# JohnsonLabJanelia/laserCalib

Hardware: NVIDIA B200
Metric: LM_iters_per_sec (higher is better)
Workload: dtype f64

## Files before the change

### include/lcba.h

```cpp
#ifndef LCBA_H
#define LCBA_H

#include <stddef.h>
#include <stdint.h>

#ifdef __cplusplus
extern "C" {
#endif

#define LCBA_VERSION 100
#define LCBA_CAM_PARAMS 11
#define LCBA_MAX_CAMERAS 64
#define LCBA_MAX_TRACE 512

enum {
  LCBA_OK = 0,
  LCBA_E_ARG = -1,
  LCBA_E_CUDA = -2,
  LCBA_E_STATE = -3,
  LCBA_E_UNSUPPORTED = -4,
  LCBA_E_NONFINITE = -5,
  LCBA_E_NCCL = -6
};

// ... 100 lines not shown

int lcba_nccl_unique_id(void* id_out128);
int lcba_comm_init(lcba_t* h, int32_t rank, int32_t nranks, const void* id128);

int lcba_debug_tr2d(double B00, double B01, double B11, double g0, double g1, double Delta,
                    double* p_out2, int* newton_out);

int lcba_debug_chol(lcba_t* h, int32_t n, const double* A, const double* rhs, double mu, const double* d,
                    int32_t grid, double* x_out, double* factor_out, int32_t* fail_out);

#define LCBA_STEP_SCALARS 18
int lcba_debug_step(lcba_t* h, double lam, double mu, int32_t mode, double* pc_out, double* pp_out,
                    double* scalars_out);

int lcba_debug_schur_stats(lcba_t* h, long long* out, int max_ctas, int* nkinds, int* nslices);

int lcba_debug_mma_plan(int32_t C, int32_t sm_count, int32_t* units_out, int32_t max_kinds,
                        int32_t* nslices_out, int32_t* ok_out);

int lcba_debug_i8_plan(int32_t C, int64_t P, int32_t sm_count, int32_t* tiles_out, int32_t max_tiles,
                       int32_t* work_out, int32_t max_work, int32_t* nwork_out, int32_t* nrg_out,
                       int64_t* nkb_out);

int lcba_debug_i8_fallback(lcba_t* h);

int lcba_debug_peer_reduce(lcba_t* h, int enable);

int lcba_host_is_nondecreasing_i64(const int64_t* v, int64_t n, int32_t threads);

#ifdef __cplusplus
}
#endif
#endif
```

### lasercalib_b200/_cabi.py

```python
from __future__ import annotations

import ctypes as C
import os

import numpy as np

_PKG = os.path.dirname(os.path.abspath(__file__))
LIB_PATH = os.path.join(_PKG, "liblcba.so")

LCBA_MAX_TRACE = 512
E_NAMES = {-1: "LCBA_E_ARG", -2: "LCBA_E_CUDA", -3: "LCBA_E_STATE", -4: "LCBA_E_UNSUPPORTED",
           -5: "LCBA_E_NONFINITE", -6: "LCBA_E_NCCL"}

SYMBOLS = ["lcba_version", "lcba_create", "lcba_destroy", "lcba_last_error", "lcba_default_options",
           "lcba_set_problem", "lcba_set_problem_shard", "lcba_set_params", "lcba_get_params", "lcba_rotate", "lcba_project",
           "lcba_unproject", "lcba_residuals", "lcba_jacobian_blocks", "lcba_sparsity_indices", "lcba_solve",
           "lcba_get_trace", "lcba_get_grad", "lcba_get_profile", "lcba_linearize",
           "lcba_time_device", "lcba_nccl_unique_id", "lcba_comm_init", "lcba_debug_tr2d",
           "lcba_sq_normal", "lcba_debug_schur_stats", "lcba_debug_mma_plan",
           "lcba_set_iteration_callback", "lcba_debug_i8_plan", "lcba_host_is_nondecreasing_i64", "lcba_debug_peer_reduce",
           "lcba_debug_i8_fallback", "lcba_debug_chol", "lcba_debug_step"]

STEP_SCALARS = ["reg_term", "Delta", "Jg2", "aa", "ab", "bb", "JAA", "JAB", "JBB", "gtgt", "gtp", "pp",
                "c0", "c1", "predicted", "step_h_norm", "step_norm", "chol_fail"]


class Options(C.Structure):
    _fields_ = [("ftol", C.c_double), ("xtol", C.c_double), ("gtol", C.c_double),
                ("max_nfev", C.c_int64), ("verbose", C.c_int32), ("profile", C.c_int32),
                ("max_iterations", C.c_int32), ("fix_cameras", C.c_int32), ("shared_intrinsics", C.c_int32), ("reserved", C.c_int32 * 3)]


class TraceRow(C.Structure):
    _fields_ = [("iteration", C.c_int64), ("nfev", C.c_int64), ("cost", C.c_double),
                ("cost_reduction", C.c_double), ("step_norm", C.c_double),
                ("optimality", C.c_double), ("delta", C.c_double), ("reg_term", C.c_double)]


class Result(C.Structure):
    _fields_ = [("cost", C.c_double), ("optimality", C.c_double), ("initial_cost", C.c_double),
                ("nfev", C.c_int64), ("njev", C.c_int64), ("iterations", C.c_int64),
                ("status", C.c_int32), ("n_trace", C.c_int32), ("solve_ms", C.c_double),
                ("gpu_launches", C.c_int64), ("reserved", C.c_double * 6)]

# ... 44 lines not shown
    lib.lcba_get_params.argtypes = [vp, vp, vp]
    lib.lcba_rotate.argtypes = [vp, i64, vp, vp, vp]
    lib.lcba_project.argtypes = [vp, i64, vp, vp, vp]
    lib.lcba_unproject.argtypes = [vp, i64, vp, vp, i64, vp, vp, vp, vp, vp]
    lib.lcba_residuals.argtypes = [vp, vp, vp, pd]
    lib.lcba_jacobian_blocks.argtypes = [vp, vp, vp, vp]
    lib.lcba_sparsity_indices.argtypes = [vp, i32, i64, i64, vp, vp, vp]
    lib.lcba_solve.argtypes = [vp, C.POINTER(Options), C.POINTER(Result)]
    lib.lcba_get_trace.argtypes = [vp, C.POINTER(TraceRow), i32]
    lib.lcba_set_iteration_callback.argtypes = [vp, ITERATION_CB, vp]
    lib.lcba_get_grad.argtypes = [vp, vp]
    lib.lcba_get_profile.argtypes = [vp, C.POINTER(KernelStat), i32, C.POINTER(i32)]
    lib.lcba_linearize.argtypes = [vp, dbl, vp, vp, vp, vp, pd]
    lib.lcba_time_device.argtypes = [vp, i32, i32, pd]
    lib.lcba_nccl_unique_id.argtypes = [vp]
    lib.lcba_comm_init.argtypes = [vp, i32, i32, vp]
    lib.lcba_sq_normal.argtypes = [vp, i32, vp, pd, vp, vp]
    lib.lcba_debug_mma_plan.argtypes = [i32, i32, vp, i32, C.POINTER(i32), C.POINTER(i32)]
    lib.lcba_debug_schur_stats.argtypes = [vp, vp, C.c_int, C.POINTER(C.c_int), C.POINTER(C.c_int)]
    lib.lcba_debug_i8_plan.argtypes = [i32, i64, i32, vp, i32, vp, i32, C.POINTER(i32), C.POINTER(i32), C.POINTER(i64)]
    lib.lcba_host_is_nondecreasing_i64.argtypes = [vp, i64, i32]
    lib.lcba_debug_peer_reduce.argtypes = [vp, i32]
    lib.lcba_debug_i8_fallback.argtypes = [vp]
    lib.lcba_debug_tr2d.argtypes = [dbl, dbl, dbl, dbl, dbl, dbl, pd, C.POINTER(C.c_int)]
    lib.lcba_debug_chol.argtypes = [vp, i32, vp, vp, dbl, vp, i32, vp, vp, C.POINTER(i32)]
    lib.lcba_debug_step.argtypes = [vp, dbl, dbl, i32, vp, vp, vp]
    _lib = lib
    return lib


def _ptr(a):
    return None if a is None else a.ctypes.data_as(C.c_void_p)


def _f64(a, shape=None):
    a = np.ascontiguousarray(a, dtype=np.float64)
    if shape is not None:
        a = a.reshape(shape)
    return a


def _i64(a):
    return np.ascontiguousarray(a, dtype=np.int64)


class Engine:
# ... 158 lines not shown
        return g

    def profile(self):
        stats = (KernelStat * 64)()
        n = C.c_int32()
        self._check(self.lib.lcba_get_profile(self.h, stats, 64, C.byref(n)))
        return {s.name.decode(): dict(launches=s.launches, total_ms=s.total_ms)
                for s in stats[:n.value]}

    def linearize(self, lam):
        n = 11 * self.C
        S = np.empty((n, n))
        rhs = np.empty(n)
        g = np.empty(n + 3 * self.P)
        sc = np.empty(n + 3 * self.P)
        cost = C.c_double()
        self._check(self.lib.lcba_linearize(self.h, float(lam), _ptr(S), _ptr(rhs), _ptr(g),
                                            _ptr(sc), C.byref(cost)))
        return dict(S=S, rhs=rhs, grad=g, scale_inv=sc, cost=cost.value)

    def i8_fell_back(self):
        return self.lib.lcba_debug_i8_fallback(self.h)

    def debug_chol(self, A, rhs, mu=0.0, d=None, grid=0):
        A = _f64(A)
        n = A.shape[0]
        if A.shape != (n, n):
            raise ValueError("A must be square")
        rhs = _f64(rhs).ravel()
        d = None if d is None else _f64(d).ravel()
        if rhs.size != n or (d is not None and d.size != n):
            raise ValueError("rhs and d must have n entries")
        x = np.empty(n)
        factor = np.empty((n + 1, n))
        fail = C.c_int32()
        self._check(self.lib.lcba_debug_chol(self.h, n, _ptr(A), _ptr(rhs), float(mu), _ptr(d), int(grid),
                                             _ptr(x), _ptr(factor), C.byref(fail)))
        return x, factor, fail.value

    STEP_FULL, STEP_FIX_CAMERAS, STEP_SHARED_INTRINSICS = 0, 1, 2

    def debug_step(self, lam, mu=0.0, mode=0):
        pc = np.empty(11 * self.C)
        pp = np.empty(3 * self.P)
        sc = np.empty(len(STEP_SCALARS))
        self._check(self.lib.lcba_debug_step(self.h, float(lam), float(mu), int(mode), _ptr(pc), _ptr(pp), _ptr(sc)))
# ... 28 lines not shown
```

### lasercalib_b200/csrc/lcba.cu

```cuda
#include <dlfcn.h>
#include <math.h>
#include <stdio.h>
#include <string.h>
#include <algorithm>
#include <map>
#include <string>
#include <thread>
#include <vector>

#include <nvtx3/nvToolsExt.h>

#include "common.cuh"
#include "control.cuh"
#include "dense.cuh"
#include "eval.cuh"
#include "ingest.cuh"
#include "linearize.cuh"
#include "dense_passes.cuh"
#include "schur.cuh"
#include "schur_mma.cuh"
#include "schur_i8.cuh"
#include "peer_reduce.cuh"
#include "variants.cuh"

// ... 504 lines not shown
  h->plan = make_schur_plan(C, h->sm_count, h->smem_optin - 2048);
  LCBA_TRY(dev_alloc(h, &h->d_kinds, h->plan.kinds.size()));
  LCBA_TRY(dev_alloc(h, &h->d_hws, h->plan.hws.size()));
  LCBA_CUDA(h, cudaMemcpyAsync(h->d_kinds, h->plan.kinds.data(), h->plan.kinds.size() * sizeof(SchurKind),
                               cudaMemcpyHostToDevice, st));
  LCBA_CUDA(h, cudaMemcpyAsync(h->d_hws, h->plan.hws.data(), h->plan.hws.size() * sizeof(SchurHw),
                               cudaMemcpyHostToDevice, st));
  LCBA_TRY(dev_alloc(h, &h->d_Sred, h->plan.part_stride));
  h->use_mma = false;
  h->d_mkinds = nullptr; h->d_U = nullptr; h->d_Upart = nullptr; h->d_Yg = nullptr;
  int max_slices = h->plan.nslices;
  {
    const char* de = getenv("LCBA_MMA_DENSITY");
    const double min_density = de ? atof(de) : 0.25;
    const bool dense = (double)h->n_pairs >= min_density * (double)P * C;
    const char* env = getenv("LCBA_SCHUR_MMA");
    const bool want = env ? atoi(env) != 0 : (dense && C >= 8);
    if (want && C <= MMA_MAX_CAMERAS) {
      {
        const char* ie = getenv("LCBA_SCHUR_I8");
        h->use_i8 = ie ? atoi(ie) != 0 : P >= 32768;
      }
      if (h->use_i8) {
        h->i8plan = make_i8_plan(C, P, h->sm_count);
        const I8Plan& ip = h->i8plan;
        h->i8_groups = (C + I8_GROUP_CAMS - 1) / I8_GROUP_CAMS;
        h->i8_gx_max = (int)std::max<long long>(1, std::min<long long>(ip.nkb, (long long)h->sm_count * 4 / h->i8_groups));
        h->i8_gx_make = (int)std::max<long long>(1, std::min<long long>(ip.nkb, (long long)h->sm_count * 3 / h->i8_groups));
        LCBA_TRY(dev_alloc(h, &h->d_i8work, ip.work.size()));
        LCBA_TRY(dev_alloc(h, &h->d_i8tiles, ip.tiles.size()));
        LCBA_CUDA(h, cudaMemcpyAsync(h->d_i8work, ip.work.data(), ip.work.size() * sizeof(I8Work), cudaMemcpyHostToDevice, st));
        LCBA_CUDA(h, cudaMemcpyAsync(h->d_i8tiles, ip.tiles.data(), ip.tiles.size() * sizeof(I8Tile), cudaMemcpyHostToDevice, st));
        LCBA_TRY(dev_alloc(h, &h->d_i8planes, ip.plane_bytes));
        {
          const char* te = getenv("LCBA_I8_TMA");
          h->i8_tma = !(te && atoi(te) == 0) && i8_encode_maps(ip, h->d_i8planes, &h->i8maps);
          if (!h->i8_tma) memset(&h->i8maps, 0, sizeof(h->i8maps));
        }
        LCBA_TRY(dev_alloc(h, &h->d_i8partial, ip.work.size() * 128 * 64));
        LCBA_TRY(dev_alloc(h, &h->d_i8rmax, (size_t)h->i8_gx_max * ip.NRG * 8));
        LCBA_TRY(dev_alloc(h, &h->d_i8erow, (size_t)ip.NRG * 8));
        LCBA_TRY(dev_alloc(h, &h->d_i8gate, 1));
        LCBA_TRY(dev_alloc(h, &h->d_i8mrow, (size_t)ip.NRG * 8));
        LCBA_CUDA(h, cudaMemsetAsync(h->d_i8gate, 0, sizeof(int), st));
        {
          const char* ge = getenv("LCBA_I8_GUARD");
          h->i8_guard = !(ge && atoi(ge) == 0);
// ... 326 lines not shown
  KL(h, "point_factor", k_point_factor<<<nblk(h->P, 256), 256, 0, h->stream>>>(
        h->d_Vg, h->d_scl_p, lam_arg, ctl_arg, h->P, h->d_Lz));
  if (h->use_mma) {
    const MmaPlan& mp = h->mplan;
    if (!h->use_dense) {
    const size_t smem_u = ((size_t)((C * CAMTAB + 1) & ~1) + (size_t)h->camn_pb * C) * 8;
    KL(h, "cam_normal", k_cam_normal<<<h->camn_grid, 256, smem_u, h->stream>>>(
          h->d_tab[w], h->d_pts[w], h->d_pair_w, h->d_pair_start, h->d_mask, h->P, C, h->camn_pb, h->d_Upart));
    KL(h, "reduce", k_reduce_cols<<<nblk(C * CAMN_VALS, RC_COLS), RC_COLS * RC_ROWS, 0, h->stream>>>(
          h->d_Upart, h->camn_grid, C * CAMN_VALS, h->d_U));
    }
    const int nt = (NCP * C + 1 + 7) / 8, last = nt - 6 * ((nt + 5) / 6 - 1);
    if (h->use_i8) {
      const I8Plan& ip = h->i8plan;
      const int RP = ip.NRG * 8;
      const size_t smem_rm = ((size_t)I8_GROUP_CAMS * CAMTAB + 192) * 4;
      KL(h, "i8_rowmax", k_i8_rowmax<<<dim3(h->i8_gx_max, h->i8_groups), 192, smem_rm, h->stream>>>(
            h->d_tab[w], h->d_pts[w], h->d_pair_w, h->d_pair_start, h->d_mask, h->d_Lz, h->P, C, RP, h->d_i8rmax));
      KL(h, "i8_rowmax", k_i8_rowexp<<<nblk(RP, 128), 128, 0, h->stream>>>(h->d_i8rmax, h->i8_gx_max, NCP * C + 1, RP,
                                                                     h->d_i8erow, h->d_i8mrow));
      KL(h, "make_Y", k_i8_make<<<dim3(h->i8_gx_make, h->i8_groups), 192, i8_make_smem_bytes(), h->stream>>>(
            h->d_tab[w], h->d_pts[w], h->d_pair_w, h->d_pair_start, h->d_mask, h->d_Lz, h->P, C, ip.NRG, h->d_i8erow,
            h->d_i8planes));
      if (h->i8_tma)
        KL(h, "schur", k_i8_syrk<true><<<(unsigned)ip.work.size(), I8_THREADS, ip.smem_bytes, h->stream>>>(
              h->i8maps, h->d_i8planes, ip.NRG, h->d_i8work, h->d_i8partial, h->d_fail, h->d_stats));
      else
        KL(h, "schur", k_i8_syrk<false><<<(unsigned)ip.work.size(), I8_THREADS, ip.smem_bytes, h->stream>>>(
              h->i8maps, h->d_i8planes, ip.NRG, h->d_i8work, h->d_i8partial, h->d_fail, h->d_stats));
      KL(h, "schur_reduce", k_i8_gather<<<dim3((unsigned)ip.tiles.size(), 16), 256, 0, h->stream>>>(
            h->d_i8partial, h->d_i8tiles, C, h->d_i8erow, pl.npairs, h->d_Sred));
      KL(h, "schur_reduce", k_add_cam_blocks<<<nblk(C * 121, 128), 128, 0, h->stream>>>(h->d_U, C, h->d_Sred));
      if (h->i8_guard) {
        KL(h, "i8_check", k_i8_check<<<1, 256, 0, h->stream>>>(h->d_i8mrow, C, h->d_Sred, h->d_i8gate));
#define LCBA_MMA_GATED(L)                                                                            \
  KL(h, "i8_fallback", (k_schur_mma<L, false><<<dim3(mp.nslices, mp.nkinds), MMA_THREADS, mp.smem_bytes, h->stream>>>( \
          nullptr, h->d_tab[w], h->d_pts[w], h->d_pair_w, h->d_pair_start, h->d_mask, h->d_Lz, h->P, h->n_pairs, C, \
          h->d_mkinds, mp.nslices, pl.part_stride, pl.npairs, h->d_Spart, nullptr, h->d_i8gate)))
        switch (last) {
          case 1: LCBA_MMA_GATED(1); break;
          case 2: LCBA_MMA_GATED(2); break;
          case 3: LCBA_MMA_GATED(3); break;
          case 4: LCBA_MMA_GATED(4); break;
          case 5: LCBA_MMA_GATED(5); break;
          default: LCBA_MMA_GATED(6); break;
        }
#undef LCBA_MMA_GATED
        KL(h, "i8_fallback", k_i8_fallback_finish<<<h->sm_count, 256, 0, h->stream>>>(
              h->d_i8gate, h->d_Spart, mp.nslices, pl.part_stride, h->d_U, C, h->d_Sred));
      }
// ... 631 lines not shown
      cudaMemcpy(&v, h->d_i8gate, sizeof(int), cudaMemcpyDeviceToHost) != cudaSuccess) return -1;
  return v;
}

extern "C" int lcba_debug_mma_plan(int32_t C, int32_t sm_count, int32_t* units_out, int32_t max_kinds,
                                   int32_t* nslices_out, int32_t* ok_out) {
  if (C < 1 || C > LCBA_MAX_CAMERAS || !units_out) return LCBA_E_ARG;
  const MmaPlan pl = make_mma_plan(C, sm_count, 227 * 1024 - 2048);
  if (ok_out) *ok_out = (pl.nkinds > 0 && C <= MMA_MAX_CAMERAS) ? 1 : 0;
  if (nslices_out) *nslices_out = pl.nslices;
  for (int k = 0; k < pl.nkinds && k < max_kinds; ++k)
    for (int w = 0; w < MMA_CONS_WARPS; ++w) {
      const MmaUnit& u = pl.kinds[k].unit[w];
      int32_t* o = units_out + ((size_t)k * MMA_CONS_WARPS + w) * 5;
      o[0] = u.tr0; o[1] = u.tc0; o[2] = u.nr; o[3] = u.nc; o[4] = u.tri;
    }
  return pl.nkinds;
}

extern "C" int lcba_debug_i8_plan(int32_t C, int64_t P, int32_t sm_count, int32_t* tiles_out, int32_t max_tiles,
                                  int32_t* work_out, int32_t max_work, int32_t* nwork_out, int32_t* nrg_out,
                                  int64_t* nkb_out) {
  if (C < 1 || C > LCBA_MAX_CAMERAS || P < 1 || !tiles_out) return LCBA_E_ARG;
  const I8Plan pl = make_i8_plan(C, P, sm_count);
  for (size_t i = 0; i < pl.tiles.size() && (int)i < max_tiles; ++i) {
    const I8Tile& t = pl.tiles[i];
    int32_t* o = tiles_out + 8 * i;
    o[0] = t.m_rg0; o[1] = t.m_nrg; o[2] = t.n_rg0; o[3] = t.n_nrg; o[4] = t.n2_rg0; o[5] = t.n2_nrg; o[6] = t.w0; o[7] = t.nw;
  }
  if (work_out)
    for (size_t i = 0; i < pl.work.size() && (int)i < max_work; ++i) {
      work_out[3 * i] = (int32_t)i; work_out[3 * i + 1] = pl.work[i].kb0; work_out[3 * i + 2] = pl.work[i].kb1;
    }
  if (nwork_out) *nwork_out = (int32_t)pl.work.size();
  if (nrg_out) *nrg_out = pl.NRG;
  if (nkb_out) *nkb_out = pl.nkb;
  return (int)pl.tiles.size();
}

extern "C" int lcba_sq_normal(lcba_t* h, int32_t mode, const double* theta, double* cost_out,
                              double* g_out, double* H_out) {
  if (!h || !h->have_problem) { set_error(h, "lcba_sq_normal: no problem set"); return LCBA_E_STATE; }
  if (!theta || (mode != LCBA_SQ_CAMONLY && mode != LCBA_SQ_TRANSFORM) || ((g_out == nullptr) != (H_out == nullptr))) {
    set_error(h, "lcba_sq_normal: bad mode, NULL theta, or only one of g / H given");
    return LCBA_E_ARG;
  }
  cudaSetDevice(h->device);
  const int C = h->C;
  const bool derivs = g_out != nullptr;
  const int K = (mode == LCBA_SQ_CAMONLY ? C * SQC_VALS : SQT_VALS) + 1;
  const int warps = sq_camonly_warps(C, h->smem_optin);
  const int threads = (mode == LCBA_SQ_CAMONLY) ? warps * 32 : SQ_THREADS;
  const int per_sm = (mode == LCBA_SQ_CAMONLY) ? 1 : 2;
  const int grid = (int)std::max<long long>(1, std::min<long long>((h->N + threads - 1) / threads,
                                                                   (long long)h->sm_count * per_sm));
  if (!h->d_sqpart || h->sq_grid < grid || h->sq_K < K) {
    LCBA_TRY(dev_alloc(h, &h->d_sqpart, (size_t)grid * K));
    LCBA_TRY(dev_alloc(h, &h->d_sqout, (size_t)K));
    if (!h->d_theta) LCBA_TRY(dev_alloc(h, &h->d_theta, 16));
    h->sq_grid = grid;
// ... 173 lines not shown
```

### lasercalib_b200/csrc/schur_i8.cuh

```cuda
#pragma once
#include <cuda.h>
#include <algorithm>
#include <vector>
#include "common.cuh"
#include "schur_mma.cuh"

namespace lcba {

constexpr int I8_NS = 6;
constexpr int I8_DMAX = 6;
constexpr int I8_ND = I8_DMAX + 1;
constexpr int I8_PTS = 21;
constexpr int I8_STAGES = 3;
constexpr int I8_FLUSH = 224;
constexpr int I8_THREADS = 192;
constexpr int I8_RG_BYTES = 512;
constexpr int I8_GROUP_CAMS = 8;
constexpr int I8_GROUP_RG = 13;
constexpr int I8_GROUP_ROWS = I8_GROUP_RG * 8;

struct I8Work {
  int m_rg0, m_nrg, n_rg0, n_nrg, n2_rg0, n2_nrg;
  int kb0, kb1;
  int map_a, map_b1, map_b2, pad;
};
constexpr int I8_MAX_MAPS = 6;
struct alignas(64) I8Maps { CUtensorMap m[I8_MAX_MAPS]; };
struct I8Tile { int m_rg0, m_nrg, n_rg0, n_nrg, n2_rg0, n2_nrg, w0, nw; };

struct I8Plan {
  int C = 0, R = 0, NRG = 0;
  long long nkb = 0;
  int map_heights[I8_MAX_MAPS] = {0, 0, 0, 0, 0, 0};
  int nmaps = 0;
  std::vector<I8Tile> tiles;
  std::vector<I8Work> work;
  size_t plane_bytes = 0, smem_bytes = 0;
};

inline I8Plan make_i8_plan(int C, long long P, int sm_count) {
  I8Plan pl;
  pl.C = C;
  pl.R = NCP * C + 1;
  pl.NRG = (pl.R + 7) / 8;
  pl.NRG += pl.NRG & 1;
  pl.nkb = (P + I8_PTS - 1) / I8_PTS;
  const int NRG = pl.NRG;
  const int nmt = (NRG + 15) / 16;
  const int last_m = NRG - 16 * (nmt - 1);
  const bool fold = nmt > 1 && last_m <= 4;
  const int nfull = fold ? nmt - 1 : nmt;
  const int col_w = fold ? 8 - last_m : 8;
  const int c0 = 16 * (nmt - 1);
  for (int mt = 0; mt < nfull; ++mt) {
    const int m0 = 16 * mt, mn = std::min(16, NRG - m0);
    for (int n0 = 0; n0 < m0 + mn; n0 += col_w) {
      const int nn = std::min(col_w, m0 + mn - n0);
      const bool last = n0 + col_w >= m0 + mn;
      I8Tile t{m0, mn, n0, nn, fold && last ? c0 : 0, fold && last ? last_m : 0, 0, 0};
      pl.tiles.push_back(t);
    }
  }
  if (fold) {
    I8Tile t{c0, last_m, c0, last_m, 0, 0, 0, 0};
    pl.tiles.push_back(t);
  }
  auto block_cost = [](int nrg) { return nrg <= 0 ? 0.0 : (nrg <= 2 ? 592.0 : (nrg <= 4 ? 812.0 : (nrg <= 6 ? 1181.0 : 1550.0))); };
  std::vector<double> cost(pl.tiles.size());
  std::vector<long long> nr(pl.tiles.size(), 1);
  for (size_t ti = 0; ti < pl.tiles.size(); ++ti) cost[ti] = 507.0 + block_cost(pl.tiles[ti].n_nrg) + block_cost(pl.tiles[ti].n2_nrg);
  for (long long left = (long long)sm_count - (long long)pl.tiles.size(); left > 0; --left) {
    size_t worst = 0;
    double tw = -1.0;
    for (size_t ti = 0; ti < pl.tiles.size(); ++ti) {
      const double tt = nr[ti] < pl.nkb ? cost[ti] / (double)nr[ti] : -1.0;
      if (tt > tw) { tw = tt; worst = ti; }
    }
    if (tw < 0.0) break;
    ++nr[worst];
  }
  for (size_t ti = 0; ti < pl.tiles.size(); ++ti) {
    I8Tile& t = pl.tiles[ti];
    const long long n = std::min<long long>(nr[ti], pl.nkb);
    t.w0 = (int)pl.work.size();
    t.nw = (int)n;
    auto map_of = [&](int h) {
      if (h == 0) return 0;
      for (int i = 0; i < pl.nmaps && i < I8_MAX_MAPS; ++i) if (pl.map_heights[i] == h) return i;
      if (pl.nmaps < I8_MAX_MAPS) pl.map_heights[pl.nmaps] = h;
      return pl.nmaps++;
    };
    const int ma = map_of(t.m_nrg), mb1 = map_of(t.n_nrg), mb2 = map_of(t.n2_nrg);
    for (long long q = 0; q < n; ++q) {
      I8Work w{t.m_rg0, t.m_nrg, t.n_rg0, t.n_nrg, t.n2_rg0, t.n2_nrg, (int)(pl.nkb * q / n), (int)(pl.nkb * (q + 1) / n),
               ma, mb1, mb2, 0};
      pl.work.push_back(w);
    }
  }
  pl.plane_bytes = (size_t)pl.nkb * I8_NS * NRG * I8_RG_BYTES;
  pl.smem_bytes = (size_t)I8_STAGES * I8_NS * (16 + 8) * I8_RG_BYTES + 1024;
  return pl;
}

inline bool i8_encode_maps(const I8Plan& pl, void* planes, I8Maps* out) {
  if (pl.nmaps <= 0 || pl.nmaps > I8_MAX_MAPS) return false;
  typedef CUresult (*EncodeFn)(CUtensorMap*, CUtensorMapDataType, cuuint32_t, void*, const cuuint64_t*, const cuuint64_t*,
                               const cuuint32_t*, const cuuint32_t*, CUtensorMapInterleave, CUtensorMapSwizzle,
                               CUtensorMapL2promotion, CUtensorMapFloatOOBfill);
  void* fn = nullptr;
  cudaDriverEntryPointQueryResult qres;
  if (cudaGetDriverEntryPoint("cuTensorMapEncodeTiled", &fn, cudaEnableDefault, &qres) != cudaSuccess || !fn ||
      qres != cudaDriverEntryPointSuccess) {
    cudaGetLastError();
    return false;
  }
  const cuuint64_t gdim[4] = {128, (cuuint64_t)pl.NRG, (cuuint64_t)I8_NS, (cuuint64_t)pl.nkb};
  const cuuint64_t gstr[3] = {(cuuint64_t)I8_RG_BYTES, (cuuint64_t)pl.NRG * I8_RG_BYTES, (cuuint64_t)I8_NS * pl.NRG * I8_RG_BYTES};
  const cuuint32_t estr[4] = {1, 1, 1, 1};
  memset(out, 0, sizeof(*out));
  for (int i = 0; i < pl.nmaps; ++i) {
    const cuuint32_t box[4] = {128, (cuuint32_t)pl.map_heights[i], (cuuint32_t)I8_NS, 1};
    const CUresult r = ((EncodeFn)fn)(&out->m[i], CU_TENSOR_MAP_DATA_TYPE_UINT32, 4, planes, gdim, gstr, box, estr,
                                      CU_TENSOR_MAP_INTERLEAVE_NONE, CU_TENSOR_MAP_SWIZZLE_NONE,
                                      CU_TENSOR_MAP_L2_PROMOTION_L2_256B, CU_TENSOR_MAP_FLOAT_OOB_FILL_NONE);
    if (r != CUDA_SUCCESS) return false;
  }
  return true;
}

__device__ __forceinline__ void i8_tma_4d(uint32_t dst, const CUtensorMap* map, int c0, int c1, int c2, int c3, uint32_t bar) {
  asm volatile("cp.async.bulk.tensor.4d.shared::cluster.global.mbarrier::complete_tx::bytes [%0], [%1, {%2, %3, %4, %5}], [%6];"
               ::"r"(dst), "l"(map), "r"(c0), "r"(c1), "r"(c2), "r"(c3), "r"(bar) : "memory");
}
__device__ __forceinline__ uint32_t i8_smem_u32(const void* p) { return (uint32_t)__cvta_generic_to_shared(p); }
__device__ __forceinline__ void i8_mbar_init(uint32_t bar, uint32_t count) {
  asm volatile("mbarrier.init.shared::cta.b64 [%0], %1;" ::"r"(bar), "r"(count) : "memory");
}
__device__ __forceinline__ void i8_mbar_expect_tx(uint32_t bar, uint32_t bytes) {
  asm volatile("mbarrier.arrive.expect_tx.shared::cta.b64 _, [%0], %1;" ::"r"(bar), "r"(bytes) : "memory");
}
__device__ __forceinline__ void i8_mbar_arrive(uint32_t bar) {
  asm volatile("mbarrier.arrive.shared::cta.b64 _, [%0];" ::"r"(bar) : "memory");
}
template <bool BACKOFF>
__device__ __forceinline__ void i8_mbar_wait(uint32_t bar, uint32_t parity, int* fail) {
  const long long t0 = clock64();
  while (true) {
    uint32_t ok;
    asm volatile("{\n\t.reg .pred p;\n\tmbarrier.try_wait.parity.shared::cta.b64 p, [%1], %2;\n\tselp.u32 %0, 1, 0, p;\n\t}"
                 : "=r"(ok) : "r"(bar), "r"(parity) : "memory");
    if (ok) return;
    if (BACKOFF) __nanosleep(128);
    if (clock64() - t0 > 6000000000LL) { atomicOr(fail, 4); asm volatile("trap;"); }
  }
}
__device__ __forceinline__ void i8_bulk_g2s(uint32_t dst, const void* src, uint32_t bytes, uint32_t bar) {
  asm volatile("cp.async.bulk.shared::cluster.global.mbarrier::complete_tx::bytes [%0], [%1], %2, [%3];"
               ::"r"(dst), "l"(src), "r"(bytes), "r"(bar) : "memory");
}
template <int COLL>
__device__ __forceinline__ void i8_mma(uint32_t tmem_d, uint64_t adesc, uint64_t bdesc, uint32_t idesc, uint32_t acc) {
#define I8_MMA_ASM(Q)                                                                                      \
  asm volatile("{\n\t.reg .pred p;\n\tsetp.ne.b32 p, %4, 0;\n\t"                                          \
               "tcgen05.mma.cta_group::1.kind::i8" Q " [%0], %1, %2, %3, {%5, %5, %5, %5}, p;\n\t}"         \
               ::"r"(tmem_d), "l"(adesc), "l"(bdesc), "r"(idesc), "r"(acc), "r"(0u) : "memory")
  if (COLL == 1) I8_MMA_ASM(".collector::a::fill");
  else if (COLL == 2) I8_MMA_ASM(".collector::a::use");
  else if (COLL == 3) I8_MMA_ASM(".collector::a::lastuse");
  else I8_MMA_ASM("");
#undef I8_MMA_ASM
}
__device__ __forceinline__ void i8_commit(uint32_t bar) {
  asm volatile("tcgen05.commit.cta_group::1.mbarrier::arrive::one.shared::cluster.b64 [%0];" ::"r"(bar) : "memory");
}
__device__ __forceinline__ bool i8_elect_one() {
  uint32_t p;
  asm volatile("{\n\t.reg .pred q;\n\telect.sync _|q, 0xffffffff;\n\tselp.u32 %0, 1, 0, q;\n\t}" : "=r"(p));
  return p != 0;
}
__device__ __forceinline__ void i8_tmem_ld16(uint32_t taddr, uint32_t (&v)[16]) {
  asm volatile("tcgen05.ld.sync.aligned.32x32b.x16.b32 "
               "{%0, %1, %2, %3, %4, %5, %6, %7, %8, %9, %10, %11, %12, %13, %14, %15}, [%16];"
               : "=r"(v[0]), "=r"(v[1]), "=r"(v[2]), "=r"(v[3]), "=r"(v[4]), "=r"(v[5]), "=r"(v[6]), "=r"(v[7]),
                 "=r"(v[8]), "=r"(v[9]), "=r"(v[10]), "=r"(v[11]), "=r"(v[12]), "=r"(v[13]), "=r"(v[14]), "=r"(v[15])
               : "r"(taddr) : "memory");
}

__device__ __forceinline__ void i8_item_values(const double* __restrict__ T, const double (&X)[3],
                                               const double (&li)[9], double w, bool live, double (&y)[3][NCP]) {
  ObsLin L;
  obs_linearize<false>(T, X[0], X[1], X[2], 0.0, 0.0, w, L, live);
  double Q[2][3];
#pragma unroll
  for (int i = 0; i < 2; ++i) {
    Q[i][0] = L.Jp[i][0] * li[0];
    Q[i][1] = fma(L.Jp[i][0], li[1], L.Jp[i][1] * li[2]);
// ... 320 lines not shown
    }
  }
}

template <bool TMA>
__global__ void __launch_bounds__(I8_THREADS, 1)
k_i8_syrk(const __grid_constant__ I8Maps maps, const unsigned char* __restrict__ planes, int NRG,
          const I8Work* __restrict__ work, double* __restrict__ partial, int* __restrict__ fail,
          long long* __restrict__ stats ) {
  extern __shared__ __align__(1024) uint8_t i8_smem[];
  __shared__ __align__(8) uint64_t s_bar[2 * I8_STAGES + 2];
  __shared__ uint32_t s_tmem;
  const I8Work W = work[blockIdx.x];
  const int tid = threadIdx.x, wid = tid >> 5, lane = tid & 31;
  const uint32_t a_bytes = (uint32_t)W.m_nrg * I8_RG_BYTES, b_bytes = (uint32_t)W.n_nrg * I8_RG_BYTES;
  const uint32_t b2_bytes = (uint32_t)W.n2_nrg * I8_RG_BYTES;
  const uint32_t B2_OFF = (uint32_t)I8_NS * b_bytes;
  constexpr uint32_t A_REGION = (uint32_t)I8_NS * 16 * I8_RG_BYTES;
  constexpr uint32_t STAGE_BYTES = (uint32_t)I8_NS * (16 + 8) * I8_RG_BYTES;
  const uint32_t smem0 = i8_smem_u32(i8_smem);
  const uint32_t bar_full = i8_smem_u32(&s_bar[0]), bar_empty = i8_smem_u32(&s_bar[I8_STAGES]);
  const uint32_t bar_tfull = i8_smem_u32(&s_bar[2 * I8_STAGES]), bar_tempty = i8_smem_u32(&s_bar[2 * I8_STAGES + 1]);
  const int ncol = W.n_nrg * 8, ncol2 = W.n2_nrg * 8;
  if (tid == 0) {
    for (int s = 0; s < I8_STAGES; ++s) { i8_mbar_init(bar_full + 8 * s, 1); i8_mbar_init(bar_empty + 8 * s, 1); }
    i8_mbar_init(bar_tfull, 1);
    i8_mbar_init(bar_tempty, 128);
    asm volatile("fence.mbarrier_init.release.cluster;" ::: "memory");
  }
  if (wid == 5) {
    asm volatile("tcgen05.alloc.cta_group::1.sync.aligned.shared::cta.b32 [%0], %1;" ::"r"(i8_smem_u32(&s_tmem)), "r"(512u) : "memory");
    asm volatile("tcgen05.relinquish_alloc_permit.cta_group::1.sync.aligned;" ::: "memory");
  }
  asm volatile("tcgen05.fence::before_thread_sync;" ::: "memory");
  __syncthreads();
  asm volatile("tcgen05.fence::after_thread_sync;" ::: "memory");
  const uint32_t tmem = s_tmem;
  const int nkb = W.kb1 - W.kb0;

  if (wid == 4) {
    if (TMA) {
      if (lane == 0) {
        for (int it = 0; it < nkb; ++it) {
          const int st = it % I8_STAGES;
          if (it >= I8_STAGES) i8_mbar_wait<false>(bar_empty + 8 * st, ((it / I8_STAGES) - 1) & 1, fail);
          i8_mbar_expect_tx(bar_full + 8 * st, (uint32_t)I8_NS * (a_bytes + b_bytes + b2_bytes));
          const uint32_t dstA = smem0 + st * STAGE_BYTES, dstB = dstA + A_REGION;
          const int kb = W.kb0 + it;
          i8_tma_4d(dstA, &maps.m[W.map_a], 0, W.m_rg0, 0, kb, bar_full + 8 * st);
          i8_tma_4d(dstB, &maps.m[W.map_b1], 0, W.n_rg0, 0, kb, bar_full + 8 * st);
          if (W.n2_nrg > 0) i8_tma_4d(dstB + B2_OFF, &maps.m[W.map_b2], 0, W.n2_rg0, 0, kb, bar_full + 8 * st);
        }
      }
    } else {
    const int ci = lane / 3, cb = lane - 3 * ci;
    const bool mine = lane < 3 * I8_NS && (cb < 2 || W.n2_nrg > 0);
    for (int it = 0; it < nkb; ++it) {
      const int st = it % I8_STAGES;
      if (it >= I8_STAGES) i8_mbar_wait<false>(bar_empty + 8 * st, ((it / I8_STAGES) - 1) & 1, fail);
      if (lane == 0) i8_mbar_expect_tx(bar_full + 8 * st, (uint32_t)I8_NS * (a_bytes + b_bytes + b2_bytes));
      __syncwarp();
      if (mine) {
        const unsigned char* src = planes + (size_t)(W.kb0 + it) * I8_NS * NRG * I8_RG_BYTES + (size_t)ci * NRG * I8_RG_BYTES;
        const uint32_t dstA = smem0 + st * STAGE_BYTES, dstB = dstA + A_REGION;
        if (cb == 0) i8_bulk_g2s(dstA + ci * a_bytes, src + (size_t)W.m_rg0 * I8_RG_BYTES, a_bytes, bar_full + 8 * st);
        else if (cb == 1) i8_bulk_g2s(dstB + ci * b_bytes, src + (size_t)W.n_rg0 * I8_RG_BYTES, b_bytes, bar_full + 8 * st);
        else i8_bulk_g2s(dstB + B2_OFF + ci * b2_bytes, src + (size_t)W.n2_rg0 * I8_RG_BYTES, b2_bytes, bar_full + 8 * st);
      }
    }
    }
  } else if (wid == 5) {
    if (i8_elect_one()) {
      int since_flush = 0, nflush = 0;
      long long t_wait = 0;
      const long long t_begin = stats ? clock64() : 0;
// ... 7 lines not shown
          const long long w0 = clock64();
          i8_mbar_wait<false>(bar_full + 8 * st, (it / I8_STAGES) & 1, fail);
          t_wait += clock64() - w0;
        } else {
          i8_mbar_wait<false>(bar_full + 8 * st, (it / I8_STAGES) & 1, fail);
        }
        asm volatile("tcgen05.fence::after_thread_sync;" ::: "memory");
        const uint32_t sA = smem0 + st * STAGE_BYTES, sB = sA + A_REGION;
        const bool first = since_flush == 0;
        const uint32_t sB2 = sB + B2_OFF;
        if (ncol2 == 0) {
          if (ncol == 64) i8_issue_block<64, 0>(first, tmem, sA, sB, sB2, a_bytes, b_bytes, b2_bytes);
          else if (ncol == 48) i8_issue_block<48, 0>(first, tmem, sA, sB, sB2, a_bytes, b_bytes, b2_bytes);
          else if (ncol == 32) i8_issue_block<32, 0>(first, tmem, sA, sB, sB2, a_bytes, b_bytes, b2_bytes);
          else i8_issue_block<16, 0>(first, tmem, sA, sB, sB2, a_bytes, b_bytes, b2_bytes);
        } else if (ncol2 == 16) {
          if (ncol == 48) i8_issue_block<48, 16>(first, tmem, sA, sB, sB2, a_bytes, b_bytes, b2_bytes);
          else if (ncol == 32) i8_issue_block<32, 16>(first, tmem, sA, sB, sB2, a_bytes, b_bytes, b2_bytes);
          else i8_issue_block<16, 16>(first, tmem, sA, sB, sB2, a_bytes, b_bytes, b2_bytes);
        } else {
          if (ncol == 32) i8_issue_block<32, 32>(first, tmem, sA, sB, sB2, a_bytes, b_bytes, b2_bytes);
          else i8_issue_block<16, 32>(first, tmem, sA, sB, sB2, a_bytes, b_bytes, b2_bytes);
        }
        i8_commit(bar_empty + 8 * st);
        ++since_flush;
        if (since_flush == I8_FLUSH || it == nkb - 1) {
          i8_commit(bar_tfull);
          since_flush = 0;
          ++nflush;
        }
      }
      if (stats) { stats[4 * blockIdx.x] = t_wait; stats[4 * blockIdx.x + 1] = clock64() - t_begin; }
    }
  } else {
    const int q = wid & 3;
    const int row = q * 32 + lane;
    double acc[64];
#pragma unroll
    for (int c = 0; c < 64; ++c) acc[c] = 0.0;
    const int nfl = (nkb + I8_FLUSH - 1) / I8_FLUSH;
    for (int f = 0; f < nfl; ++f) {
      i8_mbar_wait<true>(bar_tfull, f & 1, fail);
      asm volatile("tcgen05.fence::after_thread_sync;" ::: "memory");
#pragma unroll 1
      for (int d = 0; d < I8_ND; ++d) {
        const double sc = ldexp(1.0, -8 * (d + 2));
        const uint32_t taddr = tmem + ((uint32_t)(q * 32) << 16) + (uint32_t)(d * ncol);
#pragma unroll
        for (int h = 0; h < 4; ++h) {
          if (16 * h < ncol) {
            uint32_t v[16];
            i8_tmem_ld16(taddr + 16 * h, v);
            asm volatile("tcgen05.wait::ld.sync.aligned;" ::: "memory");
#pragma unroll
            for (int c = 0; c < 16; ++c) acc[16 * h + c] = fma((double)(int)v[c], sc, acc[16 * h + c]);
          } else if (16 * h >= 64 - ncol2) {
            uint32_t v[16];
            i8_tmem_ld16(tmem + ((uint32_t)(q * 32) << 16) + (uint32_t)(I8_ND * ncol + d * ncol2 + 16 * h - (64 - ncol2)), v);
            asm volatile("tcgen05.wait::ld.sync.aligned;" ::: "memory");
#pragma unroll
            for (int c = 0; c < 16; ++c) acc[16 * h + c] = fma((double)(int)v[c], sc, acc[16 * h + c]);
          }
        }
      }
      asm volatile("tcgen05.fence::before_thread_sync;" ::: "memory");
      i8_mbar_arrive(bar_tempty);
    }
    double* out = partial + ((size_t)blockIdx.x * 128 + row) * 64;
#pragma unroll
    for (int c = 0; c < 64; ++c) out[c] = acc[c];
  }
  asm volatile("tcgen05.fence::before_thread_sync;" ::: "memory");
  __syncthreads();
  if (wid == 5) asm volatile("tcgen05.dealloc.cta_group::1.sync.aligned.b32 %0, %1;" ::"r"(tmem), "r"(512u) : "memory");
}

__global__ void __launch_bounds__(256)
k_i8_gather(const double* __restrict__ partial, const I8Tile* __restrict__ tiles, int C,
            const int* __restrict__ e_row, int npairs, double* __restrict__ Sred) {
  const I8Tile T = tiles[blockIdx.x];
  const int n = NCP * C;
  const int nr = T.m_nrg * 8, nc1 = T.n_nrg * 8, nc2 = T.n2_nrg * 8, nc = nc1 + nc2;
  for (int idx = threadIdx.x + blockDim.x * blockIdx.y; idx < nr * nc; idx += blockDim.x * gridDim.y) {
    const int tr = idx / nc, tcl = idx - tr * nc;
    const bool second = tcl >= nc1;
    const int tc = second ? 64 - nc2 + (tcl - nc1) : tcl;
    int rho = T.m_rg0 * 8 + tr, sig = second ? T.n2_rg0 * 8 + (tcl - nc1) : T.n_rg0 * 8 + tcl;
    if (second) { const int x = rho; rho = sig; sig = x; }
    if (rho > n || sig >= n || sig > rho) continue;
    double s = 0.0;
    for (int w = 0; w < T.nw; ++w) s += partial[((size_t)(T.w0 + w) * 128 + tr) * 64 + tc];
    const double v = -ldexp(s, e_row[rho] + e_row[sig]);
    const int ck = sig / NCP, cb = sig % NCP;
    if (rho == n) { Sred[(size_t)npairs * 121 + ck * NCP + cb] = v; continue; }
    const int cj = rho / NCP, ra = rho % NCP;
    double* blk = Sred + (size_t)(cj * (cj + 1) / 2 + ck) * 121;
// ... 45 lines not shown
```

Before: 127.7.

## Multicast shared A-operand across CTA clusters and add TMA L2 prefetch in i8 SYRK

The int8 Schur SYRK kernel now pairs work items that share the same row tile and launches them as 2-CTA clusters. Each CTA loads half of the A-operand digit planes and multicasts them to its partner, and the empty barriers are signalled across the cluster with multicast commits. A TMA L2 prefetch that runs several k-blocks ahead is also added. The aim is to cut global/L2 traffic for the A operand and hide load latency. In exchange it adds cluster synchronisation, needs a scheduling check that falls back to non-clustered launches, and couples paired CTAs so that one stalls when the other does.

```diff
diff --git a/include/lcba.h b/include/lcba.h
--- a/include/lcba.h
+++ b/include/lcba.h
@@ -146,6 +146,11 @@
                        int32_t* work_out, int32_t max_work, int32_t* nwork_out, int32_t* nrg_out,
                        int64_t* nkb_out);
 
+int lcba_debug_i8_clusters(int32_t C, int64_t P, int32_t sm_count, int32_t max_cluster, int32_t* work_out,
+                           int32_t max_work, int32_t* nwork_out, int32_t* nmaps_out, int64_t* kb_bytes_out);
+
+int lcba_debug_i8_route(lcba_t* h);
+
 int lcba_debug_i8_fallback(lcba_t* h);
 
 int lcba_debug_peer_reduce(lcba_t* h, int enable);
diff --git a/lasercalib_b200/_cabi.py b/lasercalib_b200/_cabi.py
--- a/lasercalib_b200/_cabi.py
+++ b/lasercalib_b200/_cabi.py
@@ -19,7 +19,8 @@
            "lcba_time_device", "lcba_nccl_unique_id", "lcba_comm_init", "lcba_debug_tr2d",
            "lcba_sq_normal", "lcba_debug_schur_stats", "lcba_debug_mma_plan",
            "lcba_set_iteration_callback", "lcba_debug_i8_plan", "lcba_host_is_nondecreasing_i64", "lcba_debug_peer_reduce",
-           "lcba_debug_i8_fallback", "lcba_debug_chol", "lcba_debug_step"]
+           "lcba_debug_i8_fallback", "lcba_debug_chol", "lcba_debug_step",
+           "lcba_debug_i8_clusters", "lcba_debug_i8_route"]
 
 STEP_SCALARS = ["reg_term", "Delta", "Jg2", "aa", "ab", "bb", "JAA", "JAB", "JBB", "gtgt", "gtp", "pp",
                 "c0", "c1", "predicted", "step_h_norm", "step_norm", "chol_fail"]
@@ -110,6 +111,8 @@
     lib.lcba_host_is_nondecreasing_i64.argtypes = [vp, i64, i32]
     lib.lcba_debug_peer_reduce.argtypes = [vp, i32]
     lib.lcba_debug_i8_fallback.argtypes = [vp]
+    lib.lcba_debug_i8_clusters.argtypes = [i32, i64, i32, i32, vp, i32, C.POINTER(i32), C.POINTER(i32), C.POINTER(i64)]
+    lib.lcba_debug_i8_route.argtypes = [vp]
     lib.lcba_debug_tr2d.argtypes = [dbl, dbl, dbl, dbl, dbl, dbl, pd, C.POINTER(C.c_int)]
     lib.lcba_debug_chol.argtypes = [vp, i32, vp, vp, dbl, vp, i32, vp, vp, C.POINTER(i32)]
     lib.lcba_debug_step.argtypes = [vp, dbl, dbl, i32, vp, vp, vp]
@@ -314,6 +317,9 @@
     def i8_fell_back(self):
         return self.lib.lcba_debug_i8_fallback(self.h)
 
+    def i8_route(self):
+        return self.lib.lcba_debug_i8_route(self.h)
+
     def debug_chol(self, A, rhs, mu=0.0, d=None, grid=0):
         A = _f64(A)
         n = A.shape[0]
diff --git a/lasercalib_b200/csrc/lcba.cu b/lasercalib_b200/csrc/lcba.cu
--- a/lasercalib_b200/csrc/lcba.cu
+++ b/lasercalib_b200/csrc/lcba.cu
@@ -550,7 +550,17 @@
         h->use_i8 = ie ? atoi(ie) != 0 : P >= 32768;
       }
       if (h->use_i8) {
-        h->i8plan = make_i8_plan(C, P, h->sm_count);
+        h->i8plan = make_i8_plan(C, P, h->sm_count, I8_CLUSTER);
+        if (h->i8plan.cluster > 1) {
+          cudaLaunchAttribute at;
+          const cudaLaunchConfig_t cfg = i8_syrk_config(h->i8plan, st, &at);
+          int nclusters = 0;
+          if (cudaOccupancyMaxActiveClusters(&nclusters, k_i8_syrk<true>, &cfg) != cudaSuccess ||
+              (size_t)nclusters * h->i8plan.cluster < h->i8plan.work.size()) {
+            cudaGetLastError();
+            h->i8plan = make_i8_plan(C, P, h->sm_count, 1);
+          }
+        }
         const I8Plan& ip = h->i8plan;
         h->i8_groups = (C + I8_GROUP_CAMS - 1) / I8_GROUP_CAMS;
         h->i8_gx_max = (int)std::max<long long>(1, std::min<long long>(ip.nkb, (long long)h->sm_count * 4 / h->i8_groups));
@@ -923,10 +933,12 @@
       KL(h, "make_Y", k_i8_make<<<dim3(h->i8_gx_make, h->i8_groups), 192, i8_make_smem_bytes(), h->stream>>>(
             h->d_tab[w], h->d_pts[w], h->d_pair_w, h->d_pair_start, h->d_mask, h->d_Lz, h->P, C, ip.NRG, h->d_i8erow,
             h->d_i8planes));
-      if (h->i8_tma)
-        KL(h, "schur", k_i8_syrk<true><<<(unsigned)ip.work.size(), I8_THREADS, ip.smem_bytes, h->stream>>>(
-              h->i8maps, h->d_i8planes, ip.NRG, h->d_i8work, h->d_i8partial, h->d_fail, h->d_stats));
-      else
+      if (h->i8_tma) {
+        cudaLaunchAttribute at;
+        const cudaLaunchConfig_t cfg = i8_syrk_config(ip, h->stream, &at);
+        KL(h, "schur", cudaLaunchKernelEx(&cfg, k_i8_syrk<true>, h->i8maps, (const unsigned char*)h->d_i8planes, ip.NRG,
+                                          (const I8Work*)h->d_i8work, h->d_i8partial, h->d_fail, h->d_stats));
+      } else
         KL(h, "schur", k_i8_syrk<false><<<(unsigned)ip.work.size(), I8_THREADS, ip.smem_bytes, h->stream>>>(
               h->i8maps, h->d_i8planes, ip.NRG, h->d_i8work, h->d_i8partial, h->d_fail, h->d_stats));
       KL(h, "schur_reduce", k_i8_gather<<<dim3((unsigned)ip.tiles.size(), 16), 256, 0, h->stream>>>(
@@ -1604,20 +1616,41 @@
                                   int32_t* work_out, int32_t max_work, int32_t* nwork_out, int32_t* nrg_out,
                                   int64_t* nkb_out) {
   if (C < 1 || C > LCBA_MAX_CAMERAS || P < 1 || !tiles_out) return LCBA_E_ARG;
-  const I8Plan pl = make_i8_plan(C, P, sm_count);
+  const I8Plan pl = make_i8_plan(C, P, sm_count, I8_CLUSTER);
   for (size_t i = 0; i < pl.tiles.size() && (int)i < max_tiles; ++i) {
     const I8Tile& t = pl.tiles[i];
     int32_t* o = tiles_out + 8 * i;
     o[0] = t.m_rg0; o[1] = t.m_nrg; o[2] = t.n_rg0; o[3] = t.n_nrg; o[4] = t.n2_rg0; o[5] = t.n2_nrg; o[6] = t.w0; o[7] = t.nw;
   }
   if (work_out)
-    for (size_t i = 0; i < pl.work.size() && (int)i < max_work; ++i) {
-      work_out[3 * i] = (int32_t)i; work_out[3 * i + 1] = pl.work[i].kb0; work_out[3 * i + 2] = pl.work[i].kb1;
+    for (size_t i = 0; i < pl.work.size(); ++i) {
+      const int s = pl.work[i].part;
+      if (s < max_work) { work_out[3 * s] = (int32_t)i; work_out[3 * s + 1] = pl.work[i].kb0; work_out[3 * s + 2] = pl.work[i].kb1; }
     }
   if (nwork_out) *nwork_out = (int32_t)pl.work.size();
   if (nrg_out) *nrg_out = pl.NRG;
   if (nkb_out) *nkb_out = pl.nkb;
   return (int)pl.tiles.size();
+}
+
+extern "C" int lcba_debug_i8_clusters(int32_t C, int64_t P, int32_t sm_count, int32_t max_cluster, int32_t* work_out,
+                                      int32_t max_work, int32_t* nwork_out, int32_t* nmaps_out, int64_t* kb_bytes_out) {
+  if (C < 1 || C > LCBA_MAX_CAMERAS || P < 1) return LCBA_E_ARG;
+  const I8Plan pl = make_i8_plan(C, P, sm_count, max_cluster);
+  if (work_out)
+    for (size_t i = 0; i < pl.work.size() && (int)i < max_work; ++i) {
+      const I8Work& w = pl.work[i];
+      work_out[4 * i] = w.part; work_out[4 * i + 1] = w.kb0; work_out[4 * i + 2] = w.kb1; work_out[4 * i + 3] = w.share;
+    }
+  if (nwork_out) *nwork_out = (int32_t)pl.work.size();
+  if (nmaps_out) *nmaps_out = pl.nmaps;
+  if (kb_bytes_out) *kb_bytes_out = (int64_t)pl.kb_bytes;
+  return pl.cluster;
+}
+
+extern "C" int lcba_debug_i8_route(lcba_t* h) {
+  if (!h || !h->have_problem || !h->use_i8) return -1;
+  return h->i8_tma ? h->i8plan.cluster : 0;
 }
 
 extern "C" int lcba_sq_normal(lcba_t* h, int32_t mode, const double* theta, double* cost_out,
diff --git a/lasercalib_b200/csrc/schur_i8.cuh b/lasercalib_b200/csrc/schur_i8.cuh
--- a/lasercalib_b200/csrc/schur_i8.cuh
+++ b/lasercalib_b200/csrc/schur_i8.cuh
@@ -12,6 +12,9 @@
 constexpr int I8_ND = I8_DMAX + 1;
 constexpr int I8_PTS = 21;
 constexpr int I8_STAGES = 3;
+#ifndef I8_PREFETCH
+#define I8_PREFETCH 8
+#endif
 constexpr int I8_FLUSH = 224;
 constexpr int I8_THREADS = 192;
 constexpr int I8_RG_BYTES = 512;
@@ -22,23 +25,30 @@
 struct I8Work {
   int m_rg0, m_nrg, n_rg0, n_nrg, n2_rg0, n2_nrg;
   int kb0, kb1;
-  int map_a, map_b1, map_b2, pad;
+  int map_a, map_b1, map_b2;
+  int part;
+  int share;
+  int pad;
 };
-constexpr int I8_MAX_MAPS = 6;
+constexpr int I8_MAX_MAPS = 8;
+constexpr int I8_CLUSTER = 2;
 struct alignas(64) I8Maps { CUtensorMap m[I8_MAX_MAPS]; };
 struct I8Tile { int m_rg0, m_nrg, n_rg0, n_nrg, n2_rg0, n2_nrg, w0, nw; };
 
 struct I8Plan {
   int C = 0, R = 0, NRG = 0;
   long long nkb = 0;
-  int map_heights[I8_MAX_MAPS] = {0, 0, 0, 0, 0, 0};
+  int map_heights[I8_MAX_MAPS] = {};
+  int map_digits[I8_MAX_MAPS] = {};
   int nmaps = 0;
+  int cluster = 1;
   std::vector<I8Tile> tiles;
   std::vector<I8Work> work;
   size_t plane_bytes = 0, smem_bytes = 0;
+  size_t kb_bytes = 0;
 };
 
-inline I8Plan make_i8_plan(int C, long long P, int sm_count) {
+inline I8Plan make_i8_plan(int C, long long P, int sm_count, int max_cluster) {
   I8Plan pl;
   pl.C = C;
   pl.R = NCP * C + 1;
@@ -66,37 +76,62 @@
     pl.tiles.push_back(t);
   }
   auto block_cost = [](int nrg) { return nrg <= 0 ? 0.0 : (nrg <= 2 ? 592.0 : (nrg <= 4 ? 812.0 : (nrg <= 6 ? 1181.0 : 1550.0))); };
-  std::vector<double> cost(pl.tiles.size());
-  std::vector<long long> nr(pl.tiles.size(), 1);
-  for (size_t ti = 0; ti < pl.tiles.size(); ++ti) cost[ti] = 507.0 + block_cost(pl.tiles[ti].n_nrg) + block_cost(pl.tiles[ti].n2_nrg);
-  for (long long left = (long long)sm_count - (long long)pl.tiles.size(); left > 0; --left) {
+  const size_t nt = pl.tiles.size();
+  std::vector<double> cost(nt);
+  std::vector<long long> nr(nt, 1);
+  for (size_t ti = 0; ti < nt; ++ti) cost[ti] = 507.0 + block_cost(pl.tiles[ti].n_nrg) + block_cost(pl.tiles[ti].n2_nrg);
+  for (long long left = (long long)sm_count - (long long)nt; left > 0; --left) {
     size_t worst = 0;
     double tw = -1.0;
-    for (size_t ti = 0; ti < pl.tiles.size(); ++ti) {
+    for (size_t ti = 0; ti < nt; ++ti) {
       const double tt = nr[ti] < pl.nkb ? cost[ti] / (double)nr[ti] : -1.0;
       if (tt > tw) { tw = tt; worst = ti; }
     }
     if (tw < 0.0) break;
     ++nr[worst];
   }
-  for (size_t ti = 0; ti < pl.tiles.size(); ++ti) {
+  long long total = 0;
+  for (size_t ti = 0; ti < nt; ++ti) total += nr[ti] = std::min<long long>(nr[ti], pl.nkb);
+  std::vector<int> partner(nt, -1);
+  bool clustered = false;
+  if (max_cluster >= I8_CLUSTER && total % I8_CLUSTER == 0)
+    for (size_t ti = 0; ti + 1 < nt; ++ti)
+      if (partner[ti] < 0 && pl.tiles[ti + 1].m_rg0 == pl.tiles[ti].m_rg0 && nr[ti + 1] == nr[ti]) {
+        partner[ti] = (int)ti + 1;
+        partner[ti + 1] = (int)ti;
+        clustered = true;
+      }
+  pl.cluster = clustered ? I8_CLUSTER : 1;
+  auto map_of = [&](int h, int nd) {
+    if (h == 0) return 0;
+    for (int i = 0; i < pl.nmaps && i < I8_MAX_MAPS; ++i) if (pl.map_heights[i] == h && pl.map_digits[i] == nd) return i;
+    if (pl.nmaps < I8_MAX_MAPS) { pl.map_heights[pl.nmaps] = h; pl.map_digits[pl.nmaps] = nd; }
+    return pl.nmaps++;
+  };
+  std::vector<I8Work> by_tile;
+  for (size_t ti = 0; ti < nt; ++ti) {
     I8Tile& t = pl.tiles[ti];
-    const long long n = std::min<long long>(nr[ti], pl.nkb);
-    t.w0 = (int)pl.work.size();
+    const long long n = nr[ti];
+    const int a_nd = partner[ti] >= 0 ? I8_NS / I8_CLUSTER : I8_NS;
+    t.w0 = (int)by_tile.size();
     t.nw = (int)n;
-    auto map_of = [&](int h) {
-      if (h == 0) return 0;
-      for (int i = 0; i < pl.nmaps && i < I8_MAX_MAPS; ++i) if (pl.map_heights[i] == h) return i;
-      if (pl.nmaps < I8_MAX_MAPS) pl.map_heights[pl.nmaps] = h;
-      return pl.nmaps++;
-    };
-    const int ma = map_of(t.m_nrg), mb1 = map_of(t.n_nrg), mb2 = map_of(t.n2_nrg);
+    const int ma = map_of(t.m_nrg, a_nd), mb1 = map_of(t.n_nrg, I8_NS), mb2 = map_of(t.n2_nrg, I8_NS);
     for (long long q = 0; q < n; ++q) {
       I8Work w{t.m_rg0, t.m_nrg, t.n_rg0, t.n_nrg, t.n2_rg0, t.n2_nrg, (int)(pl.nkb * q / n), (int)(pl.nkb * (q + 1) / n),
-               ma, mb1, mb2, 0};
-      pl.work.push_back(w);
-    }
-  }
+               ma, mb1, mb2, (int)by_tile.size(), partner[ti] >= 0 ? (1 << I8_CLUSTER) - 1 : 0, 0};
+      by_tile.push_back(w);
+    }
+    pl.kb_bytes += (size_t)I8_RG_BYTES * (a_nd * t.m_nrg + I8_NS * (t.n_nrg + t.n2_nrg));
+  }
+  for (size_t ti = 0; ti < nt; ++ti)
+    if (partner[ti] > (int)ti)
+      for (int q = 0; q < pl.tiles[ti].nw; ++q) {
+        pl.work.push_back(by_tile[pl.tiles[ti].w0 + q]);
+        pl.work.push_back(by_tile[pl.tiles[partner[ti]].w0 + q]);
+      }
+  for (size_t ti = 0; ti < nt; ++ti)
+    if (partner[ti] < 0)
+      for (int q = 0; q < pl.tiles[ti].nw; ++q) pl.work.push_back(by_tile[pl.tiles[ti].w0 + q]);
   pl.plane_bytes = (size_t)pl.nkb * I8_NS * NRG * I8_RG_BYTES;
   pl.smem_bytes = (size_t)I8_STAGES * I8_NS * (16 + 8) * I8_RG_BYTES + 1024;
   return pl;
@@ -119,7 +154,7 @@
   const cuuint32_t estr[4] = {1, 1, 1, 1};
   memset(out, 0, sizeof(*out));
   for (int i = 0; i < pl.nmaps; ++i) {
-    const cuuint32_t box[4] = {128, (cuuint32_t)pl.map_heights[i], (cuuint32_t)I8_NS, 1};
+    const cuuint32_t box[4] = {128, (cuuint32_t)pl.map_heights[i], (cuuint32_t)pl.map_digits[i], 1};
     const CUresult r = ((EncodeFn)fn)(&out->m[i], CU_TENSOR_MAP_DATA_TYPE_UINT32, 4, planes, gdim, gstr, box, estr,
                                       CU_TENSOR_MAP_INTERLEAVE_NONE, CU_TENSOR_MAP_SWIZZLE_NONE,
                                       CU_TENSOR_MAP_L2_PROMOTION_L2_256B, CU_TENSOR_MAP_FLOAT_OOB_FILL_NONE);
@@ -128,9 +163,46 @@
   return true;
 }
 
+inline cudaLaunchConfig_t i8_syrk_config(const I8Plan& pl, cudaStream_t stream, cudaLaunchAttribute* at) {
+  at->id = cudaLaunchAttributeClusterDimension;
+  at->val.clusterDim.x = (unsigned)pl.cluster;
+  at->val.clusterDim.y = at->val.clusterDim.z = 1;
+  cudaLaunchConfig_t cfg = {};
+  cfg.gridDim = dim3((unsigned)pl.work.size());
+  cfg.blockDim = dim3(I8_THREADS);
+  cfg.dynamicSmemBytes = pl.smem_bytes;
+  cfg.stream = stream;
+  cfg.attrs = at;
+  cfg.numAttrs = 1;
+  return cfg;
+}
+
 __device__ __forceinline__ void i8_tma_4d(uint32_t dst, const CUtensorMap* map, int c0, int c1, int c2, int c3, uint32_t bar) {
   asm volatile("cp.async.bulk.tensor.4d.shared::cluster.global.mbarrier::complete_tx::bytes [%0], [%1, {%2, %3, %4, %5}], [%6];"
                ::"r"(dst), "l"(map), "r"(c0), "r"(c1), "r"(c2), "r"(c3), "r"(bar) : "memory");
+}
+__device__ __forceinline__ void i8_tma_4d_mc(uint32_t dst, const CUtensorMap* map, int c0, int c1, int c2, int c3, uint32_t bar,
+                                             uint16_t mask) {
+  asm volatile("cp.async.bulk.tensor.4d.shared::cluster.global.mbarrier::complete_tx::bytes.multicast::cluster"
+               " [%0], [%1, {%2, %3, %4, %5}], [%6], %7;"
+               ::"r"(dst), "l"(map), "r"(c0), "r"(c1), "r"(c2), "r"(c3), "r"(bar), "h"(mask) : "memory");
+}
+__device__ __forceinline__ void i8_tma_prefetch(const CUtensorMap* map, int c0, int c1, int c2, int c3) {
+  asm volatile("cp.async.bulk.prefetch.tensor.4d.L2.global.tile [%0, {%1, %2, %3, %4}];"
+               ::"l"(map), "r"(c0), "r"(c1), "r"(c2), "r"(c3) : "memory");
+}
+__device__ __forceinline__ uint32_t i8_cluster_rank() {
+  uint32_t r;
+  asm volatile("mov.u32 %0, %%cluster_ctarank;" : "=r"(r));
+  return r;
+}
+__device__ __forceinline__ uint32_t i8_cluster_size() {
+  uint32_t n;
+  asm volatile("mov.u32 %0, %%cluster_nctarank;" : "=r"(n));
+  return n;
+}
+__device__ __forceinline__ void i8_cluster_sync() {
+  asm volatile("barrier.cluster.arrive.release.aligned;\n\tbarrier.cluster.wait.acquire.aligned;" ::: "memory");
 }
 __device__ __forceinline__ uint32_t i8_smem_u32(const void* p) { return (uint32_t)__cvta_generic_to_shared(p); }
 __device__ __forceinline__ void i8_mbar_init(uint32_t bar, uint32_t count) {
@@ -172,6 +244,10 @@
 }
 __device__ __forceinline__ void i8_commit(uint32_t bar) {
   asm volatile("tcgen05.commit.cta_group::1.mbarrier::arrive::one.shared::cluster.b64 [%0];" ::"r"(bar) : "memory");
+}
+__device__ __forceinline__ void i8_commit_mc(uint32_t bar, uint16_t mask) {
+  asm volatile("tcgen05.commit.cta_group::1.mbarrier::arrive::one.shared::cluster.multicast::cluster.b64 [%0], %1;"
+               ::"r"(bar), "h"(mask) : "memory");
 }
 __device__ __forceinline__ bool i8_elect_one() {
   uint32_t p;
@@ -538,8 +614,13 @@
   const uint32_t bar_full = i8_smem_u32(&s_bar[0]), bar_empty = i8_smem_u32(&s_bar[I8_STAGES]);
   const uint32_t bar_tfull = i8_smem_u32(&s_bar[2 * I8_STAGES]), bar_tempty = i8_smem_u32(&s_bar[2 * I8_STAGES + 1]);
   const int ncol = W.n_nrg * 8, ncol2 = W.n2_nrg * 8;
+  const bool clustered = TMA && i8_cluster_size() > 1;
+  const uint32_t share = clustered ? (uint32_t)W.share : 0u;
   if (tid == 0) {
-    for (int s = 0; s < I8_STAGES; ++s) { i8_mbar_init(bar_full + 8 * s, 1); i8_mbar_init(bar_empty + 8 * s, 1); }
+    for (int s = 0; s < I8_STAGES; ++s) {
+      i8_mbar_init(bar_full + 8 * s, 1);
+      i8_mbar_init(bar_empty + 8 * s, share ? (uint32_t)__popc(share) : 1u);
+    }
     i8_mbar_init(bar_tfull, 1);
     i8_mbar_init(bar_tempty, 128);
     asm volatile("fence.mbarrier_init.release.cluster;" ::: "memory");
@@ -550,6 +631,7 @@
   }
   asm volatile("tcgen05.fence::before_thread_sync;" ::: "memory");
   __syncthreads();
+  if (clustered) i8_cluster_sync();
   asm volatile("tcgen05.fence::after_thread_sync;" ::: "memory");
   const uint32_t tmem = s_tmem;
   const int nkb = W.kb1 - W.kb0;
@@ -557,16 +639,30 @@
   if (wid == 4) {
     if (TMA) {
       if (lane == 0) {
+        const int a_nd = share ? I8_NS / __popc(share) : I8_NS;
+        const int a_d0 = share ? a_nd * __popc(share & ((1u << i8_cluster_rank()) - 1u)) : 0;
+        auto prefetch = [&](int it) {
+          const int kb = W.kb0 + it;
+          i8_tma_prefetch(&maps.m[W.map_a], 0, W.m_rg0, a_d0, kb);
+          i8_tma_prefetch(&maps.m[W.map_b1], 0, W.n_rg0, 0, kb);
+          if (W.n2_nrg > 0) i8_tma_prefetch(&maps.m[W.map_b2], 0, W.n2_rg0, 0, kb);
+        };
+        for (int it = I8_STAGES; it < min(nkb, I8_PREFETCH); ++it) prefetch(it);
         for (int it = 0; it < nkb; ++it) {
           const int st = it % I8_STAGES;
           if (it >= I8_STAGES) i8_mbar_wait<false>(bar_empty + 8 * st, ((it / I8_STAGES) - 1) & 1, fail);
+          if (it + I8_PREFETCH < nkb) prefetch(it + I8_PREFETCH);
           i8_mbar_expect_tx(bar_full + 8 * st, (uint32_t)I8_NS * (a_bytes + b_bytes + b2_bytes));
           const uint32_t dstA = smem0 + st * STAGE_BYTES, dstB = dstA + A_REGION;
           const int kb = W.kb0 + it;
-          i8_tma_4d(dstA, &maps.m[W.map_a], 0, W.m_rg0, 0, kb, bar_full + 8 * st);
+          if (share) i8_tma_4d_mc(dstA + a_d0 * a_bytes, &maps.m[W.map_a], 0, W.m_rg0, a_d0, kb, bar_full + 8 * st, (uint16_t)share);
+          else i8_tma_4d(dstA, &maps.m[W.map_a], 0, W.m_rg0, 0, kb, bar_full + 8 * st);
           i8_tma_4d(dstB, &maps.m[W.map_b1], 0, W.n_rg0, 0, kb, bar_full + 8 * st);
           if (W.n2_nrg > 0) i8_tma_4d(dstB + B2_OFF, &maps.m[W.map_b2], 0, W.n2_rg0, 0, kb, bar_full + 8 * st);
         }
+        if (share)
+          for (int it = max(nkb, I8_STAGES); it < nkb + I8_STAGES; ++it)
+            i8_mbar_wait<false>(bar_empty + 8 * (it % I8_STAGES), ((it / I8_STAGES) - 1) & 1, fail);
       }
     } else {
     const int ci = lane / 3, cb = lane - 3 * ci;
@@ -620,7 +716,8 @@
           if (ncol == 32) i8_issue_block<32, 32>(first, tmem, sA, sB, sB2, a_bytes, b_bytes, b2_bytes);
           else i8_issue_block<16, 32>(first, tmem, sA, sB, sB2, a_bytes, b_bytes, b2_bytes);
         }
-        i8_commit(bar_empty + 8 * st);
+        if (share) i8_commit_mc(bar_empty + 8 * st, (uint16_t)share);
+        else i8_commit(bar_empty + 8 * st);
         ++since_flush;
         if (since_flush == I8_FLUSH || it == nkb - 1) {
           i8_commit(bar_tfull);
@@ -628,7 +725,7 @@
           ++nflush;
         }
       }
-      if (stats) { stats[4 * blockIdx.x] = t_wait; stats[4 * blockIdx.x + 1] = clock64() - t_begin; }
+      if (stats) { stats[4 * W.part] = t_wait; stats[4 * W.part + 1] = clock64() - t_begin; }
     }
   } else {
     const int q = wid & 3;
@@ -664,12 +761,13 @@
       asm volatile("tcgen05.fence::before_thread_sync;" ::: "memory");
       i8_mbar_arrive(bar_tempty);
     }
-    double* out = partial + ((size_t)blockIdx.x * 128 + row) * 64;
+    double* out = partial + ((size_t)W.part * 128 + row) * 64;
 #pragma unroll
     for (int c = 0; c < 64; ++c) out[c] = acc[c];
   }
   asm volatile("tcgen05.fence::before_thread_sync;" ::: "memory");
   __syncthreads();
+  if (clustered) i8_cluster_sync();
   if (wid == 5) asm volatile("tcgen05.dealloc.cta_group::1.sync.aligned.b32 %0, %1;" ::"r"(tmem), "r"(512u) : "memory");
 }
 
```

Result: no change. 127.1, median of 6 (-0.5%).
